# ygtxr1997/CelebBasis

Hardware: NVIDIA H100
Metric: celeb-basis training steps/sec (SD-v1 UNet 512^2, bs=1/GPU) (higher is better)
Workload: dtype f16 operands / f32 accumulate+residual (reference: f32 with TF32 convs)

## Files before the change

### celebbasis_b200/csrc/cb_common.cuh

```cuda
#pragma once

#include <cuda.h>
#include <cuda_fp16.h>
#include <cuda_bf16.h>
#include <cuda_runtime.h>
#include <stdint.h>

#include "../../include/celebbasis_b200.h"
#include "cb_wgmma.cuh"

namespace cb {

void set_error(const char* fmt, ...);
int  check_cuda(cudaError_t e, const char* what);

#define CB_REQUIRE(cond, code, ...)                      \
    do {                                                 \
        if (!(cond)) {                                   \
            ::cb::set_error(__VA_ARGS__);                \
            return (code);                               \
        }                                                \
    } while (0)

#define CB_CUDA(call)                                                 \
// ... 188 lines not shown
        "mapa.shared::cluster.u32 ra, %0, %1;\n"
        "st.shared::cluster.v2.f32 [ra], {%2, %3};\n"
        "}\n" ::"r"(addr),
        "r"(cta), "f"(a), "f"(b)
        : "memory");
}
__device__ __forceinline__ void cluster_arrive_relaxed() { asm volatile("barrier.cluster.arrive.relaxed.aligned;" ::: "memory"); }
__device__ __forceinline__ void cluster_wait() { asm volatile("barrier.cluster.wait.acquire.aligned;" ::: "memory"); }
__device__ __forceinline__ float4 ld_shared_f32x4(uint32_t addr) {
    float4 v;
    asm volatile("ld.shared.v4.f32 {%0, %1, %2, %3}, [%4];" : "=f"(v.x), "=f"(v.y), "=f"(v.z), "=f"(v.w) : "r"(addr) : "memory");
    return v;
}

__device__ __forceinline__ uint64_t gmma_desc_sw128(uint32_t smem_addr, uint32_t lbo_bytes, uint32_t sbo_bytes) {
    uint64_t d = 0;
    d |= static_cast<uint64_t>((smem_addr & 0x3FFFFu) >> 4);
    d |= static_cast<uint64_t>((lbo_bytes >> 4) & 0x3FFFu) << 16;
    d |= static_cast<uint64_t>((sbo_bytes >> 4) & 0x3FFFu) << 32;
    d |= static_cast<uint64_t>(1) << 62;
    return d;
}

__device__ __forceinline__ float silu_f(float x) { return __fdividef(x, 1.0f + __expf(-x)); }
__device__ __forceinline__ float quick_gelu_f(float x) { return x / (1.0f + __expf(-1.702f * x)); }
__device__ __forceinline__ float gelu_f(float x) { return 0.5f * x * (1.0f + erff(x * 0.70710678118654752f)); }

template <typename T> struct cvt;
template <> struct cvt<__half> {
    static __device__ __forceinline__ float to_f(__half v) { return __half2float(v); }
    static __device__ __forceinline__ __half from_f(float v) { return __float2half_rn(v); }
};
template <> struct cvt<__nv_bfloat16> {
    static __device__ __forceinline__ float to_f(__nv_bfloat16 v) { return __bfloat162float(v); }
    static __device__ __forceinline__ __nv_bfloat16 from_f(float v) { return __float2bfloat16_rn(v); }
};
template <> struct cvt<float> {
    static __device__ __forceinline__ float to_f(float v) { return v; }
    static __device__ __forceinline__ float from_f(float v) { return v; }
};

__device__ __forceinline__ float warp_sum(float v) {
#pragma unroll
    for (int o = 16; o > 0; o >>= 1) v += __shfl_xor_sync(0xffffffffu, v, o);
    return v;
}
// ... 10 lines not shown
```

### celebbasis_b200/csrc/cb_gemm.cu

```cuda
#include <algorithm>
#include <stdarg.h>
#include <stdio.h>
#include <stdlib.h>
#include <string.h>

#include "cb_common.cuh"

namespace cb {

constexpr int BM = 128;
constexpr int BK = 64;
constexpr int kThreads = 384;

struct GemmParams {
    int M, N, K;
    int kchunks, taps, kw;
    int ksteps_last;
    int conv;
    int out_h, out_w, img_n;
    int box_w, box_h, box_i;
    int tiles_w, tiles_h;
    int stride, pad_top, pad_left;
    int b_tap_rows, flip_taps;
    void* D;
    int d_dtype;
    long long ldd, d_bs, d_bs2;
    void* D2;
    int d2_dtype;
    long long ldd2;
    int glu;
    const float* act_param;
    const float* d2_scale;
    const float* d2_shift;
    int batch_inner;
    int d_transposed;
    int vec_ok;
    int force_stages;
    const float* bias;
    int bias_row_div;
    long long ldbias;
    const void* R;
    int r_dtype;
    long long ldr, r_bs, r_bs2;
    float alpha;
    int act;
    int bf16;
    unsigned a_bytes, b_bytes;
    int splits, kiters_per_split;
    float* ws;
    unsigned* counters;
    int cluster_sk;
    int dbg_mode;
    unsigned long long* dbg;
};

template <int BN, int kStages>
struct TileCfg {
    static constexpr int kTmemCols = BN <= 64 ? 64 : (BN <= 128 ? 128 : 256);
    static constexpr int kABytes = BM * BK * 2;
    static constexpr int kBBytes = BN * BK * 2;
    static constexpr int kStageBytes = kABytes + kBBytes;
    static constexpr int kSmemBytes = kStages * kStageBytes + 1024 + 256;
    static_assert(kStages * kStageBytes >= BM * (BN + 4) * 4, "the accumulator tile is staged in the TMA ring");
};

__device__ __forceinline__ unsigned long long gtimer() {
    unsigned long long t;
    asm volatile("mov.u64 %0, %globaltimer;" : "=l"(t));
    return t;
}

__device__ __forceinline__ float apply_act(float v, int act) {
    switch (act) {
        case CB_ACT_SILU: return silu_f(v);
        case CB_ACT_GELU: return gelu_f(v);
        case CB_ACT_QUICK_GELU: return quick_gelu_f(v);
        default: return v;
    }
}

__device__ __forceinline__ void apply_act8(float (&f)[8], int act, const float* act_param, int col, int ncols = 8) {
    if (act == CB_ACT_PRELU) {
#pragma unroll
        for (int j = 0; j < 8; ++j)
            if (j < ncols) f[j] = f[j] > 0.f ? f[j] : f[j] * __ldg(act_param + col + j);
    } else {
// ... 238 lines not shown

template <int BN, bool A_MN, bool B_MN, bool BF16, int KSTEPS>
__device__ __forceinline__ void mma_batch(float (&acc)[BN / 2], uint32_t a_src, uint32_t b_src) {
    wgmma_fence();
#pragma unroll
    for (int k = 0; k < KSTEPS; ++k) {
        const uint64_t adesc = A_MN ? gmma_desc_sw128(a_src + k * 2048, 8192, 1024) : gmma_desc_sw128(a_src + k * 32, 16, 1024);
        const uint64_t bdesc = B_MN ? gmma_desc_sw128(b_src + k * 2048, 8192, 1024) : gmma_desc_sw128(b_src + k * 32, 16, 1024);
        Wgmma<BN, BF16, A_MN, B_MN>::mma(acc, adesc, bdesc, 1u);
    }
    wgmma_commit();
}

template <int BN, bool A_MN, bool B_MN, bool BF16>
__device__ __forceinline__ void mma_kiter(float (&acc)[BN / 2], uint32_t a_src, uint32_t b_src, int ksteps) {
    switch (ksteps) {
        case 4: mma_batch<BN, A_MN, B_MN, BF16, 4>(acc, a_src, b_src); break;
        case 3: mma_batch<BN, A_MN, B_MN, BF16, 3>(acc, a_src, b_src); break;
        case 2: mma_batch<BN, A_MN, B_MN, BF16, 2>(acc, a_src, b_src); break;
        default: mma_batch<BN, A_MN, B_MN, BF16, 1>(acc, a_src, b_src); break;
    }
}

template <int BN, bool kExt>
__device__ __forceinline__ void epilogue_units(const GemmParams& p, const float* stage, const long long* s_grow,
                                               const int* s_brow, const float* s_bias, int n0, int ncols_tile, int zo,
                                               int zi, int sp, uint32_t xbuf, unsigned long long* dbg) {
    constexpr int kPitch = StageCfg<BN>::kPitch;
    constexpr int G = BN / 8;
    constexpr int kResAhead = 2;
    const long long d_off = (long long)zo * p.d_bs2 + (long long)zi * p.d_bs;
    const long long r_off = (long long)zo * p.r_bs2 + (long long)zi * p.r_bs;
    const int tid = threadIdx.x;
    auto sbias_of = [&](int row, int col) { return p.bias && s_brow[row] < 0 ? s_bias + col : nullptr; };

    if (p.cluster_sk) {
        const int S = p.splits;
        const int GI = (G + S - 1) / S;
        fence_proxy_async_smem();
        cluster_sync_all();
        for (int u = tid; u < BM * G; u += kThreads) {
            const int row = u % BM, g = u / BM;
            if (g * 8 < ncols_tile) {
                const float* src = stage + row * kPitch + g * 8;
                const float4 a = *reinterpret_cast<const float4*>(src), b = *reinterpret_cast<const float4*>(src + 4);
                const uint32_t v[8] = {__float_as_uint(a.x), __float_as_uint(a.y), __float_as_uint(a.z), __float_as_uint(a.w),
// ... 71 lines not shown
#pragma unroll 1
    for (int k = 0; k < nunits; ++k) {
        if (r_pre) res_fetch(k + kResAhead, rq[kResAhead]);
        const int u = tid + k * kThreads;
        const int row = p.d_transposed ? u % BM : u / G;
        const int col = (p.d_transposed ? u / BM : u % G) * 8;
        const long long grow = s_grow[row];
        if (col < ncols_tile && grow >= 0) {
            const int ncols = min(8, ncols_tile - col);
            float f[8], r[8];
            stage_ld8(stage + row * kPitch + col, p.alpha, f);
            if (r_pre && ncols == 8) residual_unpack8(p, rq[0], r);
            epilogue_group8<kExt>(p, f, grow, s_brow[row], n0 + col, d_off, r_off, ncols, r_pre && ncols == 8 ? r : nullptr,
                                  sbias_of(row, col));
        }
        if (dbg && k == 0 && tid == 64) dbg[6] = clock64();
        if (r_pre) {
#pragma unroll
            for (int j = 0; j < kResAhead; ++j) { rq[j][0] = rq[j + 1][0]; rq[j][1] = rq[j + 1][1]; }
        }
    }
}

template <int BN, bool A_MN, bool B_MN, int kStages, bool kExt>
__global__ void __launch_bounds__(kThreads, 1)
cb_gemm_kernel(const __grid_constant__ CUtensorMap tmA, const __grid_constant__ CUtensorMap tmB,
               const __grid_constant__ GemmParams p) {
    using Cfg = TileCfg<BN, kStages>;
    using SCfg = StageCfg<BN>;
    extern __shared__ uint8_t smem_raw[];
    const uint32_t smem_base = (smem_u32(smem_raw) + 1023u) & ~1023u;
    float* stage = reinterpret_cast<float*>(smem_raw + (smem_base - smem_u32(smem_raw)));
    const uint32_t bar_base = smem_base + kStages * Cfg::kStageBytes;
    auto full_bar = [&](int s) { return bar_base + 8u * s; };
    auto empty_bar = [&](int s) { return bar_base + 8u * (kStages + s); };

    __shared__ long long s_grow[BM];
    __shared__ int s_brow[BM];
    __shared__ __align__(16) float s_bias[BN];
    const int warp = threadIdx.x >> 5;
    const int wg = __shfl_sync(0xffffffffu, warp >> 2, 0);
    if (p.dbg_mode == 3) { pdl_sync(); return; }
    unsigned long long* dbg = p.dbg ? p.dbg + 8ull * ((blockIdx.z * gridDim.y + blockIdx.y) * gridDim.x + blockIdx.x) : nullptr;
    if (dbg && threadIdx.x == 0) { dbg[0] = clock64(); dbg[7] = gtimer(); }
    const int n0 = blockIdx.x * BN;
    const int m_tile = blockIdx.y;
    const int sp = blockIdx.z % p.splits;
    const int bz = blockIdx.z / p.splits;
    const int zi = bz % p.batch_inner;
    const int zo = bz / p.batch_inner;

    int m0 = 0, ow0 = 0, oh0 = 0, img0 = 0;
    if (p.conv) {
        const int tw = m_tile % p.tiles_w;
        const int th = (m_tile / p.tiles_w) % p.tiles_h;
        const int ti = m_tile / (p.tiles_w * p.tiles_h);
        ow0 = tw * p.box_w;
        oh0 = th * p.box_h;
        img0 = ti * p.box_i;
    } else {
        m0 = m_tile * BM;
    }

    if (threadIdx.x == 0) {
        tma_prefetch_desc(&tmA);
        tma_prefetch_desc(&tmB);
        for (int s = 0; s < kStages; ++s) {
            mbar_init(full_bar(s), 1);
            mbar_init(empty_bar(s), 8);
        }
        mbar_fence_init();
        fence_proxy_async_smem();
    }
    __syncthreads();
    if (dbg && threadIdx.x == 0) dbg[1] = clock64();
    pdl_sync();

    const int kiters_all = p.dbg_mode == 1 ? 0 : p.taps * p.kchunks;
    const int it0 = sp * p.kiters_per_split;
    const int it1 = min(kiters_all, it0 + p.kiters_per_split);

    if (wg == 0) {
        if (threadIdx.x == 0) {
            int s = 0;
            uint32_t ph = 0;
            int tap = it0 / p.kchunks;
            int kc = it0 - tap * p.kchunks;
            int r = tap / p.kw;
            int sx = tap - r * p.kw;
            for (int it = it0; it < it1; ++it) {
                mbar_wait(empty_bar(s), ph ^ 1u);
                mbar_arrive_expect_tx(full_bar(s), p.a_bytes + p.b_bytes);
                const uint32_t a_dst = smem_base + s * Cfg::kStageBytes;
                const uint32_t b_dst = a_dst + Cfg::kABytes;
                const int tap_b = p.flip_taps ? (p.taps - 1 - tap) : tap;
                if (p.conv) {
                    tma_load_4d(a_dst, &tmA, full_bar(s), kc * BK, ow0 * p.stride + sx - p.pad_left,
                                oh0 * p.stride + r - p.pad_top, img0);
                } else if (A_MN) {
                    tma_load_4d(a_dst, &tmA, full_bar(s), m0, kc * BK, zi, zo);
                    tma_load_4d(a_dst + 8192, &tmA, full_bar(s), m0 + 64, kc * BK, zi, zo);
                } else {
                    tma_load_4d(a_dst, &tmA, full_bar(s), kc * BK, m0, zi, zo);
                }
                if (B_MN) {
#pragma unroll
// ... 26 lines not shown
            grow = ((long long)img * p.out_h + oh) * p.out_w + ow;
        } else {
            grow = m0 + r;
            row_valid = grow < p.M;
        }
        s_grow[r] = row_valid ? grow : -1;
        if (p.bias) {
            const long long tile_row0 = p.conv ? (((long long)img0 * p.out_h + oh0) * p.out_w + ow0) : (long long)m0;
            const long long brow0 = p.bias_row_div > 0 ? tile_row0 / p.bias_row_div : 0;
            const long long brow = p.bias_row_div > 0 ? grow / p.bias_row_div : 0;
            s_brow[r] = brow == brow0 ? -1 : static_cast<int>(brow);
            const int ncols = min(BN, p.N - n0);
            for (int i = r; i < BN; i += 128) s_bias[i] = i < ncols ? p.bias[brow0 * p.ldbias + n0 + i] : 0.f;
        }
    } else {
        float acc[BN / 2];
#pragma unroll
        for (int i = 0; i < BN / 2; ++i) acc[i] = 0.f;
        const uint32_t a_half = static_cast<uint32_t>(wg - 1) * 8192u;
        const bool releaser = (threadIdx.x & 31) == 0;
        int s = 0, s_prev = 0;
        uint32_t ph = 0;
        int kc = it0 % p.kchunks;
        for (int it = it0; it < it1; ++it) {
            mbar_wait(full_bar(s), ph);
            if (dbg && it == it0 && threadIdx.x == 128) dbg[2] = clock64();
            const uint32_t a_src = smem_base + s * Cfg::kStageBytes + a_half;
            const uint32_t b_src = smem_base + s * Cfg::kStageBytes + Cfg::kABytes;
            const int ksteps = (kc == p.kchunks - 1) ? p.ksteps_last : (BK / 16);
            wgmma_fence_regs(acc);
            if (p.bf16) mma_kiter<BN, A_MN, B_MN, true>(acc, a_src, b_src, ksteps);
            else mma_kiter<BN, A_MN, B_MN, false>(acc, a_src, b_src, ksteps);
            wgmma_wait<1>();
            wgmma_fence_regs(acc);
            if (it > it0 && releaser) mbar_arrive(empty_bar(s_prev));
            s_prev = s;
            if (++s == kStages) { s = 0; ph ^= 1u; }
            if (++kc == p.kchunks) kc = 0;
        }
        wgmma_wait<0>();
        wgmma_fence_regs(acc);
        if (it1 > it0 && releaser) mbar_arrive(empty_bar(s_prev));
        if (dbg && threadIdx.x == 128) dbg[3] = clock64();
        named_bar(4, 256);
        const int l = threadIdx.x & 31, w = warp & 3;
        float* srow = stage + ((wg - 1) * 64 + w * 16 + (l >> 2)) * SCfg::kPitch + 2 * (l & 3);
#pragma unroll
        for (int j = 0; j < BN / 8; ++j) {
            *reinterpret_cast<float2*>(srow + 8 * j) = make_float2(acc[4 * j], acc[4 * j + 1]);
            *reinterpret_cast<float2*>(srow + 8 * SCfg::kPitch + 8 * j) = make_float2(acc[4 * j + 2], acc[4 * j + 3]);
        }
    }
    named_bar(2, kThreads);
    const int ncols_tile = min(BN, p.N - n0);
    if (p.splits > 1 && !p.cluster_sk && p.dbg_mode == 0) {
        const unsigned tile_id = (static_cast<unsigned>(bz) * gridDim.y + m_tile) * gridDim.x + blockIdx.x;
        if (!splitk_reduce_to_stage<BN>(p, tile_id, sp, stage, ncols_tile)) return;
    }
    if (p.dbg_mode == 1 || p.dbg_mode == 2) return;
    if (dbg && threadIdx.x == 64) dbg[4] = clock64();
    epilogue_units<BN, kExt>(p, stage, s_grow, s_brow, s_bias, n0, ncols_tile, zo, zi, sp, smem_base + SCfg::kBytes, dbg);
    if (dbg && threadIdx.x == 64) dbg[5] = clock64();
}

typedef CUresult (*EncodeTiledFn)(CUtensorMap*, CUtensorMapDataType, cuuint32_t, void*, const cuuint64_t*,
                                  const cuuint64_t*, const cuuint32_t*, const cuuint32_t*,
                                  CUtensorMapInterleave, CUtensorMapSwizzle, CUtensorMapL2promotion,
                                  CUtensorMapFloatOOBfill);

static EncodeTiledFn get_encode_fn() {
    static EncodeTiledFn fn = nullptr;
    static bool tried = false;
    if (!tried) {
        tried = true;
        void* p = nullptr;
        cudaDriverEntryPointQueryResult q;
        if (cudaGetDriverEntryPoint("cuTensorMapEncodeTiled", &p, cudaEnableDefault, &q) == cudaSuccess &&
            q == cudaDriverEntryPointSuccess) {
            fn = reinterpret_cast<EncodeTiledFn>(p);
        }
    }
    return fn;
}

int make_tmap(CUtensorMap* out, int dtype, int rank, const void* ptr, const uint64_t* dims,
              const uint64_t* strides_bytes , const uint32_t* box, const uint32_t* estr) {
    EncodeTiledFn fn = get_encode_fn();
    CB_REQUIRE(fn != nullptr, CB_ERR_DRIVER, "cuTensorMapEncodeTiled entry point unavailable");
    CB_REQUIRE((reinterpret_cast<uintptr_t>(ptr) & 15u) == 0, CB_ERR_ALIGN, "tensor base %p not 16B aligned", ptr);
    for (int i = 0; i < rank - 1; ++i)
        CB_REQUIRE((strides_bytes[i] & 15u) == 0, CB_ERR_ALIGN, "tensor stride[%d]=%llu bytes not multiple of 16", i,
                   (unsigned long long)strides_bytes[i]);
    CUtensorMapDataType dt = dtype == CB_F16 ? CU_TENSOR_MAP_DATA_TYPE_FLOAT16 : CU_TENSOR_MAP_DATA_TYPE_BFLOAT16;
    CUresult rc = fn(out, dt, (cuuint32_t)rank, const_cast<void*>(ptr), dims, strides_bytes, box, estr,
                     CU_TENSOR_MAP_INTERLEAVE_NONE, CU_TENSOR_MAP_SWIZZLE_128B, CU_TENSOR_MAP_L2_PROMOTION_L2_256B,
                     CU_TENSOR_MAP_FLOAT_OOB_FILL_NONE);
    CB_REQUIRE(rc == CUDA_SUCCESS, CB_ERR_DRIVER,
               "cuTensorMapEncodeTiled failed rc=%d rank=%d dims=[%llu,%llu,%llu,%llu] box=[%u,%u,%u,%u]", (int)rc,
               rank, (unsigned long long)dims[0], (unsigned long long)dims[1],
               (unsigned long long)(rank > 2 ? dims[2] : 0), (unsigned long long)(rank > 3 ? dims[3] : 0), box[0],
               box[1], rank > 2 ? box[2] : 0, rank > 3 ? box[3] : 0);
    return 0;
}

static inline bool needs_ext(const GemmParams& p) { return p.D2 != nullptr || p.act == CB_ACT_PRELU || p.glu; }

template <int BN, bool A_MN, bool B_MN, int kStages, bool kExt>
static int launch_se(const CUtensorMap& tA, const CUtensorMap& tB, const GemmParams& p, dim3 grid, cudaStream_t st) {
    using Cfg = TileCfg<BN, kStages>;
    static bool attr_done = false;
    auto kern = cb_gemm_kernel<BN, A_MN, B_MN, kStages, kExt>;
    if (!attr_done) {
        CB_CUDA(cudaFuncSetAttribute(kern, cudaFuncAttributeMaxDynamicSharedMemorySize, Cfg::kSmemBytes));
        attr_done = true;
    }
    if (p.cluster_sk) {
        const int S = p.splits;
        CB_REQUIRE(S >= 2 && S <= 16 && grid.z % S == 0, CB_ERR_ARG, "cb_gemm(cluster split-K): %d slices not in [2,16]", S);
        static bool np_done = false;
        if (S > 8 && !np_done) {
            CB_CUDA(cudaFuncSetAttribute(kern, cudaFuncAttributeNonPortableClusterSizeAllowed, 1));
            np_done = true;
        }
        CB_CUDA(launch_kernel_cluster(kern, grid, dim3(kThreads), dim3(1, 1, (unsigned)S), (size_t)Cfg::kSmemBytes, st, tA, tB, p));
        CB_CUDA(cudaGetLastError());
        count_launches(1);
        return 0;
    }
CB_LAUNCH((kern), grid, kThreads, Cfg::kSmemBytes, st, tA, tB, p);
    CB_CUDA(cudaGetLastError());
    count_launches(1);
    return 0;
}

template <int BN, bool A_MN, bool B_MN, int kStages>
static int launch_s(const CUtensorMap& tA, const CUtensorMap& tB, const GemmParams& p, dim3 grid, cudaStream_t st) {
    return needs_ext(p) ? launch_se<BN, A_MN, B_MN, kStages, true>(tA, tB, p, grid, st)
                        : launch_se<BN, A_MN, B_MN, kStages, false>(tA, tB, p, grid, st);
}

static int ring_stages(int bn, const GemmParams& p, long long ctas) {
    if (bn == 256) return 4;
    static const int env_force = getenv("CB_GEMM_STAGES") ? atoi(getenv("CB_GEMM_STAGES")) : 0;
    const int force = p.force_stages ? p.force_stages : env_force;
    if (force == 3) return 3;
    if (force == 6 || ctas <= device_sm_count()) return 6;
    return 3;
}
static bool cluster_sk_fits(int bn, int splits, int stages) {
    const long long stage_bytes = ((long long)BM * (bn + 4) * 4 + 1023) / 1024 * 1024;
    const long long ring = (long long)stages * (BM * BK * 2 + bn * BK * 2);
    const long long gi = (bn / 8 + splits - 1) / splits;
    return stage_bytes + (long long)splits * gi * BM * 32 <= ring;
}

template <int BN, bool A_MN, bool B_MN>
static int launch(const CUtensorMap& tA, const CUtensorMap& tB, const GemmParams& p, dim3 grid, cudaStream_t st) {
    if constexpr (BN == 256) {
        return launch_s<BN, A_MN, B_MN, 4>(tA, tB, p, grid, st);
    } else {
        const long long ctas = (long long)grid.x * grid.y * grid.z;
        if (ring_stages(BN, p, ctas) == 6) return launch_s<BN, A_MN, B_MN, 6>(tA, tB, p, grid, st);
        return launch_s<BN, A_MN, B_MN, 3>(tA, tB, p, grid, st);
    }
}

static double tile_time_us(int bn, long long tiles, int kiters, int sms) {
    const double t_iter = (128.0 + bn) * 128.0 / 80e3;
    const long long waves = (tiles + sms - 1) / sms;
    return (double)waves * kiters * t_iter;
}

static int pick_bn(const cb_gemm_desc& d, int m_tiles, int kiters, bool requested = true) {
    const int N = d.N;
    const int sms = device_sm_count();
    int cands[3];
    int nc = 0;
    if (d.b_major == CB_MAJOR_MN) {
        if (N <= 64) return 64;
        cands[nc++] = 128;
        cands[nc++] = 64;
    } else {
        if (N <= 64) return 64;
        cands[nc++] = 160;
        cands[nc++] = 128;
// ... 31 lines not shown
    }
    CB_REQUIRE(d.N > 0 && d.K > 0 && d.batch > 0, CB_ERR_ARG, "cb_gemm: bad N/K/batch");
    CB_REQUIRE(d.d_dtype >= CB_F16 && d.d_dtype <= CB_F32, CB_ERR_ARG, "cb_gemm: bad d_dtype");
    const int es = 2;
    const bool a_mn = d.a_major == CB_MAJOR_MN, b_mn = d.b_major == CB_MAJOR_MN;
    CB_REQUIRE(!(d.conv && a_mn), CB_ERR_ARG, "cb_gemm: conv mode needs K-major A (NHWC)");
    CB_REQUIRE(!(a_mn && !b_mn), CB_ERR_ARG, "cb_gemm: (A MN-major, B K-major) is not instantiated");

    const int b_in = d.batch_inner > 0 ? d.batch_inner : d.batch;
    CB_REQUIRE(d.batch % b_in == 0, CB_ERR_ARG, "cb_gemm: batch %d not a multiple of batch_inner %d", d.batch, b_in);
    const int b_out = d.batch / b_in;
    GemmParams p;
    memset(&p, 0, sizeof(p));
    p.batch_inner = b_in;
    p.N = d.N;
    p.K = d.K;
    p.kchunks = ceil_div(d.K, BK);
    p.ksteps_last = ceil_div(d.K - (p.kchunks - 1) * BK, 16);
    p.conv = d.conv;
    p.taps = 1;
    p.kw = 1;
    p.b_tap_rows = d.b_tap_rows;
    p.flip_taps = d.flip_taps;

    CUtensorMap tA, tB;
    int m_tiles;
    if (d.conv) {
        CB_REQUIRE(d.img_n > 0 && d.img_h > 0 && d.img_w > 0 && d.out_h > 0 && d.out_w > 0 && d.kh > 0 && d.kw > 0,
                   CB_ERR_ARG, "cb_gemm(conv): bad geometry");
        CB_REQUIRE(d.stride == 1 || d.stride == 2, CB_ERR_ARG, "cb_gemm(conv): stride must be 1 or 2");
        CB_REQUIRE(d.batch == 1, CB_ERR_ARG, "cb_gemm(conv): batch must be 1 (images are rows)");
        p.taps = d.kh * d.kw;
        p.kw = d.kw;
        p.M = d.img_n * d.out_h * d.out_w;
        p.out_h = d.out_h;
        p.out_w = d.out_w;
        p.img_n = d.img_n;
        p.stride = d.stride;
        p.pad_top = d.pad_top;
        p.pad_left = d.pad_left;
        int bw = d.out_w < BM ? d.out_w : BM;
        int bh = BM / bw;
        if (bh > d.out_h) bh = d.out_h;
        int bi = BM / (bw * bh);
        if (bi > d.img_n) bi = d.img_n;
        if (bi < 1) bi = 1;
        p.box_w = bw;
        p.box_h = bh;
        p.box_i = bi;
        p.tiles_w = ceil_div(d.out_w, bw);
        p.tiles_h = ceil_div(d.out_h, bh);
        m_tiles = p.tiles_w * p.tiles_h * ceil_div(d.img_n, bi);
        p.a_bytes = (unsigned)(bw * bh * bi) * BK * es;
        const uint64_t C = (uint64_t)d.K;
        const uint64_t rowstride = (uint64_t)d.lda;
        uint64_t dims[4] = {C, (uint64_t)d.img_w, (uint64_t)d.img_h, (uint64_t)d.img_n};
        uint64_t strides[3] = {rowstride * es, rowstride * es * d.img_w, rowstride * es * d.img_w * d.img_h};
        uint32_t box[4] = {BK, (uint32_t)(bw * d.stride), (uint32_t)(bh * d.stride), (uint32_t)bi};
        uint32_t estr[4] = {1, (uint32_t)d.stride, (uint32_t)d.stride, 1};
        CB_REQUIRE(box[1] <= 256 && box[2] <= 256, CB_ERR_ARG, "cb_gemm(conv): box too large");
        int rc = make_tmap(&tA, d.ab_dtype, 4, d.A, dims, strides, box, estr);
        if (rc) return rc;
    } else {
        CB_REQUIRE(d.M > 0, CB_ERR_ARG, "cb_gemm: bad M");
        p.M = d.M;
        m_tiles = ceil_div(d.M, BM);
        p.a_bytes = BM * BK * es;
        const uint64_t dflt = (uint64_t)(a_mn ? d.lda * (int64_t)d.K : d.lda * (int64_t)d.M);
        const uint64_t bs = (uint64_t)(b_in > 1 ? d.a_batch_stride : dflt);
        const uint64_t bs2 = (uint64_t)(b_out > 1 ? d.a_batch_stride2 : dflt);
        if (a_mn) {
            uint64_t dims[4] = {(uint64_t)d.M, (uint64_t)d.K, (uint64_t)b_in, (uint64_t)b_out};
            uint64_t strides[3] = {(uint64_t)d.lda * es, bs * es, bs2 * es};
            uint32_t box[4] = {64, BK, 1, 1};
            uint32_t estr[4] = {1, 1, 1, 1};
            int rc = make_tmap(&tA, d.ab_dtype, 4, d.A, dims, strides, box, estr);
            if (rc) return rc;
        } else {
            uint64_t dims[4] = {(uint64_t)d.K, (uint64_t)d.M, (uint64_t)b_in, (uint64_t)b_out};
            uint64_t strides[3] = {(uint64_t)d.lda * es, bs * es, bs2 * es};
            uint32_t box[4] = {BK, BM, 1, 1};
            uint32_t estr[4] = {1, 1, 1, 1};
            int rc = make_tmap(&tA, d.ab_dtype, 4, d.A, dims, strides, box, estr);
            if (rc) return rc;
        }
    }

    int BN = pick_bn(d, m_tiles, p.taps * p.kchunks);
    if (d.glu && BN % 64 != 0) BN = 128;
    const int b_box_rows = BN;
    p.b_bytes = (unsigned)b_box_rows * BK * es;
    {
        const uint64_t brows_total = (uint64_t)(d.conv ? (int64_t)p.taps * d.b_tap_rows : (b_mn ? d.K : d.N));
        const uint64_t dflt = (uint64_t)(d.ldb * (int64_t)brows_total);
        const uint64_t bs = (uint64_t)(b_in > 1 ? d.b_batch_stride : dflt);
        const uint64_t bs2 = (uint64_t)(b_out > 1 ? d.b_batch_stride2 : dflt);
        uint32_t estr[4] = {1, 1, 1, 1};
        if (b_mn) {
            uint64_t dims[4] = {(uint64_t)d.N, brows_total, (uint64_t)b_in, (uint64_t)b_out};
            uint64_t strides[3] = {(uint64_t)d.ldb * es, bs * es, bs2 * es};
            uint32_t box[4] = {64, BK, 1, 1};
            int rc = make_tmap(&tB, d.ab_dtype, 4, d.B, dims, strides, box, estr);
            if (rc) return rc;
        } else {
            uint64_t dims[4] = {(uint64_t)d.K, brows_total, (uint64_t)b_in, (uint64_t)b_out};
            uint64_t strides[3] = {(uint64_t)d.ldb * es, bs * es, bs2 * es};
            uint32_t box[4] = {BK, (uint32_t)b_box_rows, 1, 1};
            int rc = make_tmap(&tB, d.ab_dtype, 4, d.B, dims, strides, box, estr);
            if (rc) return rc;
        }
    }

    p.D = d.D;
    p.d_dtype = d.d_dtype;
    p.ldd = d.ldd;
    p.d_bs = d.d_batch_stride;
    p.d_bs2 = d.d_batch_stride2;
    p.d_transposed = d.d_transposed;
    p.D2 = d.D2;
    p.d2_dtype = d.d2_dtype;
    p.ldd2 = d.ldd2;
// ... 22 lines not shown
    p.alpha = d.alpha;
    p.act = d.act;
    p.dbg = reinterpret_cast<unsigned long long*>(d.debug_timeline);
    {
        static const int mode = getenv("CB_GEMM_DBG_MODE") ? atoi(getenv("CB_GEMM_DBG_MODE")) : 0;
        p.dbg_mode = mode;
    }
    p.bf16 = d.ab_dtype == CB_BF16 ? 1 : 0;
    {
        const int des = d.d_dtype == CB_F32 ? 4 : 2;
        bool ok = ((reinterpret_cast<uintptr_t>(d.D) & 15u) == 0) && ((d.ldd * des) % 16 == 0) &&
                  ((d.d_batch_stride * des) % 16 == 0) && ((d.d_batch_stride2 * des) % 16 == 0);
        if (d.R) {
            const int res = d.r_dtype == CB_F32 ? 4 : 2;
            ok = ok && ((reinterpret_cast<uintptr_t>(d.R) & 15u) == 0) && ((d.ldr * res) % 16 == 0) &&
                 ((d.r_batch_stride * res) % 16 == 0) && ((d.r_batch_stride2 * res) % 16 == 0);
        }
        if (d.bias) ok = ok && ((reinterpret_cast<uintptr_t>(d.bias) & 15u) == 0) && ((d.ldbias * 4) % 16 == 0);
        p.vec_ok = ok ? 1 : 0;
    }

    p.force_stages = (d.stages == 3 || d.stages == 6) ? d.stages : 0;
    p.splits = 1;
    p.kiters_per_split = p.taps * p.kchunks;
    {
        const int kiters = p.taps * p.kchunks;
        const int sms = device_sm_count();
        const int bn_s = pick_bn(d, m_tiles, kiters, false);
        const long long tiles_s = (long long)ceil_div(d.N, bn_s) * m_tiles * d.batch;
        const long long counters_bytes = 65536;
        const long long avail = d.splitk_ws_bytes - counters_bytes;
        const long long tiles_max = (long long)ceil_div(d.N, 64) * m_tiles * d.batch;
        const long long slice_bytes = (long long)(d.N + 255) * m_tiles * d.batch * BM * 4;
        if (d.splitk_ws != nullptr && !d.glu && tiles_max <= counters_bytes / 4 &&
            (d.splits > 0 || (tiles_s < sms && kiters >= 8))) {
            const double out_elems = (double)p.M * d.batch * d.N;
            double best_t = tile_time_us(bn_s, tiles_s, kiters, sms);
            int best_sp = 1;
            if (d.splits > 0) {
                best_sp = d.splits < kiters ? d.splits : kiters;
            } else {
                const int max_sp = (int)(sms / tiles_s) < 64 ? (int)(sms / tiles_s) : 64;
                for (int sp = 2; sp <= max_sp; ++sp) {
                    const int per = ceil_div(kiters, sp);
                    if (per < 4) break;
                    const double t = per * ((128.0 + bn_s) * 128.0 / 80e3) + out_elems * sp / 150e3 + 3.0;
                    if (t < best_t) { best_t = t; best_sp = sp; }
                }
            }
            if (best_sp > 1) {
                const int per = ceil_div(kiters, best_sp);
                const int splits = ceil_div(kiters, per);
                if (slice_bytes * splits <= avail) {
                    p.splits = splits;
                    p.kiters_per_split = per;
                    p.counters = reinterpret_cast<unsigned*>(d.splitk_ws);
                    p.ws = reinterpret_cast<float*>(reinterpret_cast<char*>(d.splitk_ws) + counters_bytes);
                }
            }
        }
    }
    cudaStream_t st = reinterpret_cast<cudaStream_t>(stream);
    dim3 grid((unsigned)ceil_div(d.N, BN), (unsigned)m_tiles, (unsigned)(d.batch * p.splits));
    p.cluster_sk = (d.splitk_cluster == 1 && p.splits >= 2 && p.splits <= 16 && p.dbg_mode == 0 &&
                    cluster_sk_fits(BN, p.splits, ring_stages(BN, p, (long long)grid.x * grid.y * grid.z))) ? 1 : 0;
    if (!a_mn && !b_mn) {
        if (BN == 64) return launch<64, false, false>(tA, tB, p, grid, st);
        if (BN == 128) return launch<128, false, false>(tA, tB, p, grid, st);
        if (BN == 256) return launch<256, false, false>(tA, tB, p, grid, st);
        return launch<160, false, false>(tA, tB, p, grid, st);
    } else if (!a_mn && b_mn) {
        if (BN == 64) return launch<64, false, true>(tA, tB, p, grid, st);
        if (BN == 256) return launch<256, false, true>(tA, tB, p, grid, st);
        return launch<128, false, true>(tA, tB, p, grid, st);
    } else {
        if (BN == 64) return launch<64, true, true>(tA, tB, p, grid, st);
        return launch<128, true, true>(tA, tB, p, grid, st);
    }
}
```

### celebbasis_b200/vae_engine.py

```python
import torch

from . import ops
from .ops import Geo
from .unet_engine import _Attn, _round_up


class VAEEncoderEngine:
    def __init__(self, ddconfig, embed_dim, state_dict, device, *, prefix="", dtype=torch.float16,
                 res_dtype=torch.float32):
        self.dev = torch.device(device)
        self.dt = dtype
        self.rt = res_dtype
        sd, p = state_dict, prefix
        f32 = lambda t: ops.to_device(t, self.dev)
        w16 = lambda t: ops.to_device(t, self.dev, self.dt)
        pack = lambda k, **kw: ops.pack_conv_weight(sd[p + k], self.dt, device=self.dev, **kw)
        ch, mult, nres = ddconfig["ch"], ddconfig["ch_mult"], ddconfig["num_res_blocks"]
        self.in_ch = ddconfig["in_channels"]
        self.in_pad = _round_up(self.in_ch, 8)
        self.zc2 = 2 * ddconfig["z_channels"] if ddconfig.get("double_z", True) else ddconfig["z_channels"]
        self.conv_in_w, self.conv_in_b = pack("encoder.conv_in.weight", cin_pad=self.in_pad), f32(sd[p + "encoder.conv_in.bias"])
        self.ch0 = ch

        def res(pre, cin, cout):
# ... 26 lines not shown
        self.mid1 = res(p + "encoder.mid.block_1.", bin_, bin_)
        self.mid2 = res(p + "encoder.mid.block_2.", bin_, bin_)
        ak = p + "encoder.mid.attn_1."
        c = bin_
        self.attn = {"c": c, "gn": f32(sd[ak + "norm.weight"]), "bn": f32(sd[ak + "norm.bias"]),
                     "wqkv": w16(torch.cat([sd[ak + "q.weight"].reshape(c, c), sd[ak + "k.weight"].reshape(c, c),
                                            sd[ak + "v.weight"].reshape(c, c)], 0)),
                     "bqkv": f32(torch.cat([sd[ak + "q.bias"], sd[ak + "k.bias"], sd[ak + "v.bias"]], 0)),
                     "wo": w16(sd[ak + "proj_out.weight"].reshape(c, c)), "bo": f32(sd[ak + "proj_out.bias"])}
        self.no_g, self.no_b = f32(sd[p + "encoder.norm_out.weight"]), f32(sd[p + "encoder.norm_out.bias"])
        self.c_last = bin_
        self.out_rows = _round_up(self.zc2, 16)
        self.conv_out_w = pack("encoder.conv_out.weight", cout_pad=self.out_rows)
        cb = torch.zeros(self.out_rows, dtype=torch.float32, device=self.dev)
        cb[: self.zc2] = f32(sd[p + "encoder.conv_out.bias"])
        self.conv_out_b = cb
        qw = sd[p + "quant_conv.weight"]
        self.q_out = qw.shape[0]
        qpad = torch.zeros(self.q_out, _round_up(self.zc2, 8), dtype=torch.float32)
        qpad[:, : self.zc2] = qw.reshape(self.q_out, self.zc2)
        self.quant_w, self.quant_b = w16(qpad), f32(sd[p + "quant_conv.bias"])
        self.mid_pad = _round_up(self.zc2, 8)

    def _res(self, w, x, geo):
        a, _ = ops.groupnorm(x, geo, w["g1"], w["b1"], eps=1e-6, silu=True, out_dtype=self.dt)
        h, _ = ops.conv2d(a, geo, w["w1"], w["cout"], bias=w["c1b"], out_dtype=self.dt)
        b, _ = ops.groupnorm(h, geo, w["g2"], w["b2"], eps=1e-6, silu=True, out_dtype=self.dt)
        if w["ws"] is None:
            resid = x
        else:
            x16 = x if x.dtype == self.dt else ops.cast(x, self.dt)
            resid = ops.linear(x16, w["ws"], w["bs"], out_dtype=self.rt)
        out, _ = ops.conv2d(b, geo, w["w2"], w["cout"], bias=w["c2b"], out_dtype=self.rt, residual=resid)
        return out

    def _attn(self, x, geo):
        w = self.attn
        c = w["c"]
        n, _ = ops.groupnorm(x, geo, w["gn"], w["bn"], eps=1e-6, silu=False, out_dtype=self.dt)
        qkv = ops.linear(n, w["wqkv"], w["bqkv"])
        o = torch.empty(geo.rows, c, dtype=self.dt, device=self.dev)
        _Attn.fwd(qkv[:, :c], qkv[:, c:2 * c], qkv[:, 2 * c:], images=geo.n, heads=1, dh=c, nq=geo.hw, nk=geo.hw,
                  scale=float(c) ** -0.5, out=o)
        return ops.linear(o, w["wo"], w["bo"], out_dtype=self.rt, residual=x)

    @torch.no_grad()
    def encode_moments(self, x):
        x16, geo = ops.nchw_to_nhwc(x.contiguous().float(), self.in_pad, self.dt)
        h, _ = ops.conv2d(x16, geo, self.conv_in_w, self.ch0, bias=self.conv_in_b, out_dtype=self.rt)
        for blocks, down in self.levels:
            for w in blocks:
                h = self._res(w, h, geo)
            if down is not None:
                h16 = h if h.dtype == self.dt else ops.cast(h, self.dt)
                h, geo = ops.conv2d(h16, geo, down["w"], down["c"], bias=down["b"], stride=2, pad=(0, 1, 0, 1),
                                    out_dtype=self.rt)
        h = self._res(self.mid1, h, geo)
        h = self._attn(h, geo)
        h = self._res(self.mid2, h, geo)
        a, _ = ops.groupnorm(h, geo, self.no_g, self.no_b, eps=1e-6, silu=True, out_dtype=self.dt)
        m = torch.zeros(geo.rows, self.mid_pad, dtype=self.dt, device=self.dev) if self.mid_pad != self.zc2 else \
            torch.empty(geo.rows, self.mid_pad, dtype=self.dt, device=self.dev)
        ops.conv2d(a, geo, self.conv_out_w, self.zc2, bias=self.conv_out_b, out=m, cout_rows=self.out_rows)
        q = ops.linear(m, self.quant_w, self.quant_b, out_dtype=torch.float32)
        return ops.nhwc_to_nchw(q, geo, self.q_out)


class VAEDecoderEngine:

    def __init__(self, ddconfig, embed_dim, state_dict, device, *, prefix="", dtype=torch.float16, res_dtype=None):
        self.dev = torch.device(device)
        self.dt = dtype
        self.rt = res_dtype or dtype
        sd, p = state_dict, prefix
        f32 = lambda t: ops.to_device(t, self.dev)
        w16 = lambda t: ops.to_device(t, self.dev, self.dt)
        ch, mult, nres = ddconfig["ch"], ddconfig["ch_mult"], ddconfig["num_res_blocks"]
        zc = ddconfig["z_channels"]
        self.zc, self.zpad = zc, _round_up(zc, 8)
        self.out_ch = ddconfig["out_ch"]
# ... 30 lines not shown
                     "wqkv": w16(torch.cat([sd[ak + "q.weight"].reshape(c, c), sd[ak + "k.weight"].reshape(c, c),
                                            sd[ak + "v.weight"].reshape(c, c)], 0)),
                     "bqkv": f32(torch.cat([sd[ak + "q.bias"], sd[ak + "k.bias"], sd[ak + "v.bias"]], 0)),
                     "wo": w16(sd[ak + "proj_out.weight"].reshape(c, c)), "bo": f32(sd[ak + "proj_out.bias"])}
        self.levels = []
        for i in reversed(range(len(mult))):
            bout = ch * mult[i]
            blocks = []
            for j in range(nres + 1):
                blocks.append(res(p + f"decoder.up.{i}.block.{j}.", bin_, bout))
                bin_ = bout
            up = None
            if i != 0:
                uk = p + f"decoder.up.{i}.upsample.conv."
                up = {"w": ops.pack_conv_weight(sd[uk + "weight"], self.dt, device=self.dev), "b": f32(sd[uk + "bias"]), "c": bin_}
            self.levels.append((blocks, up))
        self.no_g, self.no_b = f32(sd[p + "decoder.norm_out.weight"]), f32(sd[p + "decoder.norm_out.bias"])
        self.out_rows = 16
        self.conv_out_w = ops.pack_conv_weight(sd[p + "decoder.conv_out.weight"], self.dt, device=self.dev, cout_pad=self.out_rows)
        cb = torch.zeros(self.out_rows, dtype=torch.float32, device=self.dev)
        cb[: self.out_ch] = f32(sd[p + "decoder.conv_out.bias"])
        self.conv_out_b = cb

    _res = VAEEncoderEngine._res
    _attn = VAEEncoderEngine._attn

    @torch.no_grad()
    def decode(self, z):
        z16, geo = ops.nchw_to_nhwc(z.contiguous().float(), self.zpad, self.dt)
        h0 = ops.linear(z16, self.pq_w, self.pq_b)
        h, _ = ops.conv2d(h0, geo, self.conv_in_w, self.c_in, bias=self.conv_in_b, out_dtype=self.rt)
        h = self._res(self.mid1, h, geo)
        h = self._attn(h, geo)
        h = self._res(self.mid2, h, geo)
        for blocks, up in self.levels:
            for w in blocks:
                h = self._res(w, h, geo)
            if up is not None:
                h16 = h if h.dtype == self.dt else ops.cast(h, self.dt)
                u, geo = ops.upsample2x(h16, geo)
                h, _ = ops.conv2d(u, geo, up["w"], up["c"], bias=up["b"], out_dtype=self.rt)
        a, _ = ops.groupnorm(h, geo, self.no_g, self.no_b, eps=1e-6, silu=True, out_dtype=self.dt)
        y, _ = ops.conv2d(a, geo, self.conv_out_w, self.out_ch, bias=self.conv_out_b, out_dtype=torch.float32,
                          cout_rows=self.out_rows)
        return ops.nhwc_to_nchw(y, geo, self.out_ch)
```

Measured before the change: 56.72.

## Add tap-packed conv GEMM kernel for K=8 3x3 convs and dual-dtype VAE outputs

Adds a dedicated kernel path for 3x3 stride-1 convolutions with only 8 input channels. All nine taps are loaded in one unswizzled TMA batch and issued as back-to-back wgmma ops, so the K=8 input is no longer padded to a 64-wide K chunk per tap. Separately, the pipeline-stage choice no longer depends on CTA count; it now defaults to 6 stages. The VAE encoder also emits an f16 copy of block outputs via out2 so later shortcut and downsample convs skip a separate cast kernel. The tap path relies on a hand-built no-swizzle descriptor layout and zero-filled slot, which is correctness-sensitive.

After: 58.06, median of 6. 1.02x the previous value.

```diff
diff --git a/celebbasis_b200/csrc/cb_common.cuh b/celebbasis_b200/csrc/cb_common.cuh
--- a/celebbasis_b200/csrc/cb_common.cuh
+++ b/celebbasis_b200/csrc/cb_common.cuh
@@ -234,6 +234,14 @@
     return d;
 }
 
+__device__ __forceinline__ uint64_t gmma_desc_noswz(uint32_t smem_addr, uint32_t lbo_bytes, uint32_t sbo_bytes) {
+    uint64_t d = 0;
+    d |= static_cast<uint64_t>((smem_addr & 0x3FFFFu) >> 4);
+    d |= static_cast<uint64_t>((lbo_bytes >> 4) & 0x3FFFu) << 16;
+    d |= static_cast<uint64_t>((sbo_bytes >> 4) & 0x3FFFu) << 32;
+    return d;
+}
+
 __device__ __forceinline__ float silu_f(float x) { return __fdividef(x, 1.0f + __expf(-x)); }
 __device__ __forceinline__ float quick_gelu_f(float x) { return x / (1.0f + __expf(-1.702f * x)); }
 __device__ __forceinline__ float gelu_f(float x) { return 0.5f * x * (1.0f + erff(x * 0.70710678118654752f)); }
diff --git a/celebbasis_b200/csrc/cb_gemm.cu b/celebbasis_b200/csrc/cb_gemm.cu
--- a/celebbasis_b200/csrc/cb_gemm.cu
+++ b/celebbasis_b200/csrc/cb_gemm.cu
@@ -11,6 +11,8 @@
 constexpr int BM = 128;
 constexpr int BK = 64;
 constexpr int kThreads = 384;
+constexpr int kTapSlots = 10;
+constexpr int kTapSlotA = BM * 16;
 
 struct GemmParams {
     int M, N, K;
@@ -54,14 +56,16 @@
     unsigned long long* dbg;
 };
 
-template <int BN, int kStages>
+template <int BN, int kStages, bool kTap = false>
 struct TileCfg {
     static constexpr int kTmemCols = BN <= 64 ? 64 : (BN <= 128 ? 128 : 256);
-    static constexpr int kABytes = BM * BK * 2;
-    static constexpr int kBBytes = BN * BK * 2;
+    static constexpr int kABytes = kTap ? kTapSlots * kTapSlotA : BM * BK * 2;
+    static constexpr int kBBytes = kTap ? kTapSlots * BN * 16 : BN * BK * 2;
     static constexpr int kStageBytes = kABytes + kBBytes;
-    static constexpr int kSmemBytes = kStages * kStageBytes + 1024 + 256;
-    static_assert(kStages * kStageBytes >= BM * (BN + 4) * 4, "the accumulator tile is staged in the TMA ring");
+    static constexpr int kAccBytes = (BM * (BN + 4) * 4 + 1023) / 1024 * 1024;
+    static constexpr int kRingBytes = kStages * kStageBytes >= kAccBytes ? kStages * kStageBytes : kAccBytes;
+    static constexpr int kSmemBytes = kRingBytes + 1024 + 256;
+    static_assert(kTap || kStages * kStageBytes >= BM * (BN + 4) * 4, "the accumulator tile is staged in the TMA ring");
 };
 
 __device__ __forceinline__ unsigned long long gtimer() {
@@ -346,6 +350,18 @@
     }
 }
 
+template <int BN, bool BF16>
+__device__ __forceinline__ void mma_batch_taps(float (&acc)[BN / 2], uint32_t a_src, uint32_t b_src) {
+    wgmma_fence();
+#pragma unroll
+    for (int t = 0; t < kTapSlots - 1; ++t) {
+        const uint64_t adesc = gmma_desc_noswz(a_src + t * kTapSlotA, (kTapSlots - 1 - t) * kTapSlotA, 128);
+        const uint64_t bdesc = gmma_desc_noswz(b_src + t * BN * 16, BN * 16, 128);
+        Wgmma<BN, BF16, false, false>::mma(acc, adesc, bdesc, 1u);
+    }
+    wgmma_commit();
+}
+
 template <int BN, bool kExt>
 __device__ __forceinline__ void epilogue_units(const GemmParams& p, const float* stage, const long long* s_grow,
                                                const int* s_brow, const float* s_bias, int n0, int ncols_tile, int zo,
@@ -463,16 +479,14 @@
     }
 }
 
-template <int BN, bool A_MN, bool B_MN, int kStages, bool kExt>
-__global__ void __launch_bounds__(kThreads, 1)
-cb_gemm_kernel(const __grid_constant__ CUtensorMap tmA, const __grid_constant__ CUtensorMap tmB,
-               const __grid_constant__ GemmParams p) {
-    using Cfg = TileCfg<BN, kStages>;
+template <int BN, bool A_MN, bool B_MN, int kStages, bool kExt, bool kTap>
+__device__ __forceinline__ void gemm_tile(const CUtensorMap& tmA, const CUtensorMap& tmB, const GemmParams& p) {
+    using Cfg = TileCfg<BN, kStages, kTap>;
     using SCfg = StageCfg<BN>;
     extern __shared__ uint8_t smem_raw[];
     const uint32_t smem_base = (smem_u32(smem_raw) + 1023u) & ~1023u;
     float* stage = reinterpret_cast<float*>(smem_raw + (smem_base - smem_u32(smem_raw)));
-    const uint32_t bar_base = smem_base + kStages * Cfg::kStageBytes;
+    const uint32_t bar_base = smem_base + Cfg::kRingBytes;
     auto full_bar = [&](int s) { return bar_base + 8u * s; };
     auto empty_bar = [&](int s) { return bar_base + 8u * (kStages + s); };
 
@@ -513,6 +527,13 @@
         mbar_fence_init();
         fence_proxy_async_smem();
     }
+    if constexpr (kTap) {
+        if (wg == 0) {
+            *reinterpret_cast<uint4*>(reinterpret_cast<uint8_t*>(stage) + (kTapSlots - 1) * kTapSlotA + threadIdx.x * 16) =
+                make_uint4(0u, 0u, 0u, 0u);
+            fence_proxy_async_smem();
+        }
+    }
     __syncthreads();
     if (dbg && threadIdx.x == 0) dbg[1] = clock64();
     pdl_sync();
@@ -522,7 +543,14 @@
     const int it1 = min(kiters_all, it0 + p.kiters_per_split);
 
     if (wg == 0) {
-        if (threadIdx.x == 0) {
+        if (kTap && threadIdx.x == 0 && it1 > it0) {
+            mbar_arrive_expect_tx(full_bar(0), p.a_bytes + p.b_bytes);
+            for (int t = 0, r = 0, sx = 0; t < p.taps; ++t) {
+                tma_load_4d(smem_base + t * kTapSlotA, &tmA, full_bar(0), 0, ow0 + sx - p.pad_left, oh0 + r - p.pad_top, img0);
+                if (++sx == p.kw) { sx = 0; ++r; }
+            }
+            tma_load_3d(smem_base + Cfg::kABytes, &tmB, full_bar(0), 0, n0, 0);
+        } else if (!kTap && threadIdx.x == 0) {
             int s = 0;
             uint32_t ph = 0;
             int tap = it0 / p.kchunks;
@@ -595,7 +623,14 @@
         int s = 0, s_prev = 0;
         uint32_t ph = 0;
         int kc = it0 % p.kchunks;
-        for (int it = it0; it < it1; ++it) {
+        if (kTap && it1 > it0) {
+            mbar_wait(full_bar(0), 0);
+            wgmma_fence_regs(acc);
+            const uint32_t a_src = smem_base + static_cast<uint32_t>(wg - 1) * 64u * 16u;
+            if (p.bf16) mma_batch_taps<BN, true>(acc, a_src, smem_base + Cfg::kABytes);
+            else mma_batch_taps<BN, false>(acc, a_src, smem_base + Cfg::kABytes);
+        }
+        for (int it = it0; it < (kTap ? it0 : it1); ++it) {
             mbar_wait(full_bar(s), ph);
             if (dbg && it == it0 && threadIdx.x == 128) dbg[2] = clock64();
             const uint32_t a_src = smem_base + s * Cfg::kStageBytes + a_half;
@@ -613,7 +648,7 @@
         }
         wgmma_wait<0>();
         wgmma_fence_regs(acc);
-        if (it1 > it0 && releaser) mbar_arrive(empty_bar(s_prev));
+        if (!kTap && it1 > it0 && releaser) mbar_arrive(empty_bar(s_prev));
         if (dbg && threadIdx.x == 128) dbg[3] = clock64();
         named_bar(4, 256);
         const int l = threadIdx.x & 31, w = warp & 3;
@@ -634,6 +669,20 @@
     if (dbg && threadIdx.x == 64) dbg[4] = clock64();
     epilogue_units<BN, kExt>(p, stage, s_grow, s_brow, s_bias, n0, ncols_tile, zo, zi, sp, smem_base + SCfg::kBytes, dbg);
     if (dbg && threadIdx.x == 64) dbg[5] = clock64();
+}
+
+template <int BN, bool A_MN, bool B_MN, int kStages, bool kExt>
+__global__ void __launch_bounds__(kThreads, 1)
+cb_gemm_kernel(const __grid_constant__ CUtensorMap tmA, const __grid_constant__ CUtensorMap tmB,
+               const __grid_constant__ GemmParams p) {
+    gemm_tile<BN, A_MN, B_MN, kStages, kExt, false>(tmA, tmB, p);
+}
+
+template <int BN, bool kExt>
+__global__ void __launch_bounds__(kThreads, 1)
+cb_gemm_tap_kernel(const __grid_constant__ CUtensorMap tmA, const __grid_constant__ CUtensorMap tmB,
+                   const __grid_constant__ GemmParams p) {
+    gemm_tile<BN, false, false, 1, kExt, true>(tmA, tmB, p);
 }
 
 typedef CUresult (*EncodeTiledFn)(CUtensorMap*, CUtensorMapDataType, cuuint32_t, void*, const cuuint64_t*,
@@ -656,8 +705,9 @@
     return fn;
 }
 
-int make_tmap(CUtensorMap* out, int dtype, int rank, const void* ptr, const uint64_t* dims,
-              const uint64_t* strides_bytes , const uint32_t* box, const uint32_t* estr) {
+static int make_tmap_sw(CUtensorMap* out, int dtype, int rank, const void* ptr, const uint64_t* dims,
+                       const uint64_t* strides_bytes , const uint32_t* box, const uint32_t* estr,
+                       CUtensorMapSwizzle swizzle) {
     EncodeTiledFn fn = get_encode_fn();
     CB_REQUIRE(fn != nullptr, CB_ERR_DRIVER, "cuTensorMapEncodeTiled entry point unavailable");
     CB_REQUIRE((reinterpret_cast<uintptr_t>(ptr) & 15u) == 0, CB_ERR_ALIGN, "tensor base %p not 16B aligned", ptr);
@@ -666,7 +716,7 @@
                    (unsigned long long)strides_bytes[i]);
     CUtensorMapDataType dt = dtype == CB_F16 ? CU_TENSOR_MAP_DATA_TYPE_FLOAT16 : CU_TENSOR_MAP_DATA_TYPE_BFLOAT16;
     CUresult rc = fn(out, dt, (cuuint32_t)rank, const_cast<void*>(ptr), dims, strides_bytes, box, estr,
-                     CU_TENSOR_MAP_INTERLEAVE_NONE, CU_TENSOR_MAP_SWIZZLE_128B, CU_TENSOR_MAP_L2_PROMOTION_L2_256B,
+                     CU_TENSOR_MAP_INTERLEAVE_NONE, swizzle, CU_TENSOR_MAP_L2_PROMOTION_L2_256B,
                      CU_TENSOR_MAP_FLOAT_OOB_FILL_NONE);
     CB_REQUIRE(rc == CUDA_SUCCESS, CB_ERR_DRIVER,
                "cuTensorMapEncodeTiled failed rc=%d rank=%d dims=[%llu,%llu,%llu,%llu] box=[%u,%u,%u,%u]", (int)rc,
@@ -676,13 +726,20 @@
     return 0;
 }
 
+int make_tmap(CUtensorMap* out, int dtype, int rank, const void* ptr, const uint64_t* dims,
+              const uint64_t* strides_bytes , const uint32_t* box, const uint32_t* estr) {
+    return make_tmap_sw(out, dtype, rank, ptr, dims, strides_bytes, box, estr, CU_TENSOR_MAP_SWIZZLE_128B);
+}
+
 static inline bool needs_ext(const GemmParams& p) { return p.D2 != nullptr || p.act == CB_ACT_PRELU || p.glu; }
 
-template <int BN, bool A_MN, bool B_MN, int kStages, bool kExt>
+template <int BN, bool A_MN, bool B_MN, int kStages, bool kExt, bool kTap = false>
 static int launch_se(const CUtensorMap& tA, const CUtensorMap& tB, const GemmParams& p, dim3 grid, cudaStream_t st) {
-    using Cfg = TileCfg<BN, kStages>;
+    using Cfg = TileCfg<BN, kStages, kTap>;
     static bool attr_done = false;
-    auto kern = cb_gemm_kernel<BN, A_MN, B_MN, kStages, kExt>;
+    void (*kern)(const CUtensorMap, const CUtensorMap, const GemmParams);
+    if constexpr (kTap) kern = cb_gemm_tap_kernel<BN, kExt>;
+    else kern = cb_gemm_kernel<BN, A_MN, B_MN, kStages, kExt>;
     if (!attr_done) {
         CB_CUDA(cudaFuncSetAttribute(kern, cudaFuncAttributeMaxDynamicSharedMemorySize, Cfg::kSmemBytes));
         attr_done = true;
@@ -706,19 +763,17 @@
     return 0;
 }
 
-template <int BN, bool A_MN, bool B_MN, int kStages>
+template <int BN, bool A_MN, bool B_MN, int kStages, bool kTap = false>
 static int launch_s(const CUtensorMap& tA, const CUtensorMap& tB, const GemmParams& p, dim3 grid, cudaStream_t st) {
-    return needs_ext(p) ? launch_se<BN, A_MN, B_MN, kStages, true>(tA, tB, p, grid, st)
-                        : launch_se<BN, A_MN, B_MN, kStages, false>(tA, tB, p, grid, st);
-}
-
-static int ring_stages(int bn, const GemmParams& p, long long ctas) {
+    return needs_ext(p) ? launch_se<BN, A_MN, B_MN, kStages, true, kTap>(tA, tB, p, grid, st)
+                        : launch_se<BN, A_MN, B_MN, kStages, false, kTap>(tA, tB, p, grid, st);
+}
+
+static int ring_stages(int bn, const GemmParams& p) {
     if (bn == 256) return 4;
     static const int env_force = getenv("CB_GEMM_STAGES") ? atoi(getenv("CB_GEMM_STAGES")) : 0;
     const int force = p.force_stages ? p.force_stages : env_force;
-    if (force == 3) return 3;
-    if (force == 6 || ctas <= device_sm_count()) return 6;
-    return 3;
+    return force == 3 ? 3 : 6;
 }
 static bool cluster_sk_fits(int bn, int splits, int stages) {
     const long long stage_bytes = ((long long)BM * (bn + 4) * 4 + 1023) / 1024 * 1024;
@@ -732,8 +787,7 @@
     if constexpr (BN == 256) {
         return launch_s<BN, A_MN, B_MN, 4>(tA, tB, p, grid, st);
     } else {
-        const long long ctas = (long long)grid.x * grid.y * grid.z;
-        if (ring_stages(BN, p, ctas) == 6) return launch_s<BN, A_MN, B_MN, 6>(tA, tB, p, grid, st);
+        if (ring_stages(BN, p) == 6) return launch_s<BN, A_MN, B_MN, 6>(tA, tB, p, grid, st);
         return launch_s<BN, A_MN, B_MN, 3>(tA, tB, p, grid, st);
     }
 }
@@ -811,6 +865,7 @@
     p.kw = 1;
     p.b_tap_rows = d.b_tap_rows;
     p.flip_taps = d.flip_taps;
+    const bool tap_pack = d.conv && d.K == 8 && d.kh == 3 && d.kw == 3 && d.stride == 1 && !d.flip_taps && !b_mn;
 
     CUtensorMap tA, tB;
     int m_tiles;
@@ -848,7 +903,12 @@
         uint32_t box[4] = {BK, (uint32_t)(bw * d.stride), (uint32_t)(bh * d.stride), (uint32_t)bi};
         uint32_t estr[4] = {1, (uint32_t)d.stride, (uint32_t)d.stride, 1};
         CB_REQUIRE(box[1] <= 256 && box[2] <= 256, CB_ERR_ARG, "cb_gemm(conv): box too large");
-        int rc = make_tmap(&tA, d.ab_dtype, 4, d.A, dims, strides, box, estr);
+        if (tap_pack) {
+            box[0] = 8;
+            p.a_bytes = (unsigned)(p.taps * bw * bh * bi * 16);
+        }
+        int rc = make_tmap_sw(&tA, d.ab_dtype, 4, d.A, dims, strides, box, estr,
+                              tap_pack ? CU_TENSOR_MAP_SWIZZLE_NONE : CU_TENSOR_MAP_SWIZZLE_128B);
         if (rc) return rc;
     } else {
         CB_REQUIRE(d.M > 0, CB_ERR_ARG, "cb_gemm: bad M");
@@ -875,7 +935,8 @@
         }
     }
 
-    int BN = pick_bn(d, m_tiles, p.taps * p.kchunks);
+    const int kiters = tap_pack ? 1 : p.taps * p.kchunks;
+    int BN = pick_bn(d, m_tiles, kiters);
     if (d.glu && BN % 64 != 0) BN = 128;
     const int b_box_rows = BN;
     p.b_bytes = (unsigned)b_box_rows * BK * es;
@@ -885,7 +946,14 @@
         const uint64_t bs = (uint64_t)(b_in > 1 ? d.b_batch_stride : dflt);
         const uint64_t bs2 = (uint64_t)(b_out > 1 ? d.b_batch_stride2 : dflt);
         uint32_t estr[4] = {1, 1, 1, 1};
-        if (b_mn) {
+        if (tap_pack) {
+            uint64_t dims[3] = {8, (uint64_t)d.b_tap_rows, (uint64_t)p.taps};
+            uint64_t strides[2] = {(uint64_t)d.ldb * es, (uint64_t)d.ldb * es * d.b_tap_rows};
+            uint32_t box[3] = {8, (uint32_t)BN, (uint32_t)kTapSlots};
+            p.b_bytes = (unsigned)(kTapSlots * BN * 16);
+            int rc = make_tmap_sw(&tB, d.ab_dtype, 3, d.B, dims, strides, box, estr, CU_TENSOR_MAP_SWIZZLE_NONE);
+            if (rc) return rc;
+        } else if (b_mn) {
             uint64_t dims[4] = {(uint64_t)d.N, brows_total, (uint64_t)b_in, (uint64_t)b_out};
             uint64_t strides[3] = {(uint64_t)d.ldb * es, bs * es, bs2 * es};
             uint32_t box[4] = {64, BK, 1, 1};
@@ -954,9 +1022,8 @@
 
     p.force_stages = (d.stages == 3 || d.stages == 6) ? d.stages : 0;
     p.splits = 1;
-    p.kiters_per_split = p.taps * p.kchunks;
+    p.kiters_per_split = kiters;
     {
-        const int kiters = p.taps * p.kchunks;
         const int sms = device_sm_count();
         const int bn_s = pick_bn(d, m_tiles, kiters, false);
         const long long tiles_s = (long long)ceil_div(d.N, bn_s) * m_tiles * d.batch;
@@ -995,7 +1062,13 @@
     cudaStream_t st = reinterpret_cast<cudaStream_t>(stream);
     dim3 grid((unsigned)ceil_div(d.N, BN), (unsigned)m_tiles, (unsigned)(d.batch * p.splits));
     p.cluster_sk = (d.splitk_cluster == 1 && p.splits >= 2 && p.splits <= 16 && p.dbg_mode == 0 &&
-                    cluster_sk_fits(BN, p.splits, ring_stages(BN, p, (long long)grid.x * grid.y * grid.z))) ? 1 : 0;
+                    cluster_sk_fits(BN, p.splits, ring_stages(BN, p))) ? 1 : 0;
+    if (tap_pack) {
+        if (BN == 64) return launch_s<64, false, false, 1, true>(tA, tB, p, grid, st);
+        if (BN == 128) return launch_s<128, false, false, 1, true>(tA, tB, p, grid, st);
+        if (BN == 256) return launch_s<256, false, false, 1, true>(tA, tB, p, grid, st);
+        return launch_s<160, false, false, 1, true>(tA, tB, p, grid, st);
+    }
     if (!a_mn && !b_mn) {
         if (BN == 64) return launch<64, false, false>(tA, tB, p, grid, st);
         if (BN == 128) return launch<128, false, false>(tA, tB, p, grid, st);
diff --git a/celebbasis_b200/vae_engine.py b/celebbasis_b200/vae_engine.py
--- a/celebbasis_b200/vae_engine.py
+++ b/celebbasis_b200/vae_engine.py
@@ -72,16 +72,25 @@
         self.quant_w, self.quant_b = w16(qpad), f32(sd[p + "quant_conv.bias"])
         self.mid_pad = _round_up(self.zc2, 8)
 
-    def _res(self, w, x, geo):
+    def _copy16(self, geo, c, needed):
+        if not needed or self.rt == self.dt:
+            return None
+        return torch.empty(geo.rows, c, dtype=self.dt, device=self.dev)
+
+    def _as16(self, x, x16=None):
+        if x16 is not None:
+            return x16
+        return x if x.dtype == self.dt else ops.cast(x, self.dt)
+
+    def _res(self, w, x, geo, x16=None, out16=None):
         a, _ = ops.groupnorm(x, geo, w["g1"], w["b1"], eps=1e-6, silu=True, out_dtype=self.dt)
         h, _ = ops.conv2d(a, geo, w["w1"], w["cout"], bias=w["c1b"], out_dtype=self.dt)
         b, _ = ops.groupnorm(h, geo, w["g2"], w["b2"], eps=1e-6, silu=True, out_dtype=self.dt)
         if w["ws"] is None:
             resid = x
         else:
-            x16 = x if x.dtype == self.dt else ops.cast(x, self.dt)
-            resid = ops.linear(x16, w["ws"], w["bs"], out_dtype=self.rt)
-        out, _ = ops.conv2d(b, geo, w["w2"], w["cout"], bias=w["c2b"], out_dtype=self.rt, residual=resid)
+            resid = ops.linear(self._as16(x, x16), w["ws"], w["bs"], out_dtype=self.rt)
+        out, _ = ops.conv2d(b, geo, w["w2"], w["cout"], bias=w["c2b"], out_dtype=self.rt, residual=resid, out2=out16)
         return out
 
     def _attn(self, x, geo):
@@ -97,15 +106,22 @@
     @torch.no_grad()
     def encode_moments(self, x):
         x16, geo = ops.nchw_to_nhwc(x.contiguous().float(), self.in_pad, self.dt)
-        h, _ = ops.conv2d(x16, geo, self.conv_in_w, self.ch0, bias=self.conv_in_b, out_dtype=self.rt)
+        nxt = [b for blocks, _ in self.levels for b in blocks] + [self.mid1]
+        h16 = self._copy16(geo, self.ch0, nxt[0]["ws"] is not None)
+        h, _ = ops.conv2d(x16, geo, self.conv_in_w, self.ch0, bias=self.conv_in_b, out_dtype=self.rt, out2=h16)
+        k = 0
         for blocks, down in self.levels:
-            for w in blocks:
-                h = self._res(w, h, geo)
+            for j, w in enumerate(blocks):
+                k += 1
+                o16 = self._copy16(geo, w["cout"], down is not None if j + 1 == len(blocks) else nxt[k]["ws"] is not None)
+                h, h16 = self._res(w, h, geo, x16=h16, out16=o16), o16
             if down is not None:
-                h16 = h if h.dtype == self.dt else ops.cast(h, self.dt)
-                h, geo = ops.conv2d(h16, geo, down["w"], down["c"], bias=down["b"], stride=2, pad=(0, 1, 0, 1),
-                                    out_dtype=self.rt)
-        h = self._res(self.mid1, h, geo)
+                ogeo = Geo(geo.n, geo.h // 2, geo.w // 2)
+                o16 = self._copy16(ogeo, down["c"], nxt[k]["ws"] is not None)
+                h, geo = ops.conv2d(self._as16(h, h16), geo, down["w"], down["c"], bias=down["b"], stride=2,
+                                    pad=(0, 1, 0, 1), out_dtype=self.rt, out2=o16)
+                h16 = o16
+        h = self._res(self.mid1, h, geo, x16=h16)
         h = self._attn(h, geo)
         h = self._res(self.mid2, h, geo)
         a, _ = ops.groupnorm(h, geo, self.no_g, self.no_b, eps=1e-6, silu=True, out_dtype=self.dt)
@@ -182,6 +198,7 @@
         cb[: self.out_ch] = f32(sd[p + "decoder.conv_out.bias"])
         self.conv_out_b = cb
 
+    _as16 = VAEEncoderEngine._as16
     _res = VAEEncoderEngine._res
     _attn = VAEEncoderEngine._attn
 
```
